# eather0056/Catenary-Model-Estimation-and-MPC-Control-for-ROV-Tethered-Systems

Measured on AMD Instinct MI355X. Metric: MPC rollouts/sec (horizon-steps/sec) at N=20, K=4096; 1/2/4/8 GPU, higher is better.
Workload: dtype f64

## Files before the change

### catenary-model-estimation-and-mpc-control-for-rov-tethered-systems_amd/csrc/rollout_kernels.h

```cpp
#pragma once
#include "device_math.h"

namespace rovmpc {

constexpr int MODEL_BUILTIN = 0;
constexpr int MODEL_INTERP  = 1;
constexpr int MODEL_JIT     = 2;

#ifndef ROVMPC_JIT_FMAP
#define ROVMPC_JIT_FMAP 0
#endif
#ifndef ROVMPC_JIT_N
#define ROVMPC_JIT_N 0
#endif
#ifndef ROVMPC_JIT_CKC
#define ROVMPC_JIT_CKC 0
#endif
#ifndef ROVMPC_JIT_USED
#define ROVMPC_JIT_USED 0xffffffffu
#endif

#ifndef ROVMPC_JIT_NSUB
#define ROVMPC_JIT_NSUB 0
#endif
// ... 61 lines not shown
    int ck_shift;
    unsigned used_planes;
    unsigned magic_3n;
    unsigned long long *granules;
    unsigned epoch;
    int sweeper;
    double *result;
    long long *slots;
    long long k_offset;
    int rank, world;
    unsigned long long *stamps;
    unsigned long long samp_seed, samp_step;
    double samp_mean[3], samp_std[3];
    const double *samp_warm;
    double *samp_best;
    double *samp_blk_u;
    double samp_state[ROVMPC_STATE_LEN];
    T *gtab;
    unsigned long long *gtab_tag;
};


template <typename T>
RV_DEV T interp_eval(const int32_t *__restrict__ code, int n, const T *__restrict__ consts,
                     const T *feat, int fstride, T *stack, int sstride) {
    T top = T(0);
    int sp = 0;
    for (int pc = 0; pc < n; ++pc) {
        int ins = code[pc];
        int op = ins & 0xff, arg = ins >> 8;
        switch (op) {
// ... 27 lines not shown
        case ROVMPC_OP_SAFE_LOG: top = m_log(m_abs(top) + T(1e-5)); break;
        case ROVMPC_OP_SAFE_SQRT: top = m_sqrt(m_abs(top)); break;
        default: top = m_nan<T>(); break;
        }
    }
    return top;
}

constexpr unsigned ERR_WAIT_ROLLED = 1;
constexpr unsigned ERR_CONSUMED    = 2;
constexpr unsigned ERR_SWEEP       = 4;
RV_DEV void raise_error(unsigned *err, unsigned bit) {
    if (err) __hip_atomic_fetch_or(err, bit, __ATOMIC_RELAXED, __HIP_MEMORY_SCOPE_SYSTEM);
}

RV_DEV void st_agent(double *p, double v) { __hip_atomic_store(p, v, __ATOMIC_RELAXED, __HIP_MEMORY_SCOPE_AGENT); }
RV_DEV void st_agent(long long *p, long long v) { __hip_atomic_store(p, v, __ATOMIC_RELAXED, __HIP_MEMORY_SCOPE_AGENT); }
RV_DEV void st_agent(unsigned long long *p, unsigned long long v) { __hip_atomic_store(p, v, __ATOMIC_RELAXED, __HIP_MEMORY_SCOPE_AGENT); }
RV_DEV unsigned long long ld_agent(const unsigned long long *p) { return __hip_atomic_load(p, __ATOMIC_RELAXED, __HIP_MEMORY_SCOPE_AGENT); }
constexpr int GRAN = 4;
RV_DEV void publish_traj_ready(unsigned long long *granules, int nblocks, unsigned epoch) {
    st_agent(granules + 3 * (size_t)nblocks + blockIdx.x, (unsigned long long)epoch << 32);
}
RV_DEV void publish_best(unsigned long long *granules, int nblocks, unsigned epoch, double cost, unsigned lane) {
    const unsigned long long bits = (unsigned long long)__double_as_longlong(cost), tag = (unsigned long long)epoch << 32;
    st_agent(granules + blockIdx.x, tag | (bits >> 32));
    st_agent(granules + nblocks + blockIdx.x, tag | (bits & 0xffffffffULL));
    st_agent(granules + 2 * (size_t)nblocks + blockIdx.x, tag | lane);
}
RV_DEV double ld_agent(const double *p) { return __hip_atomic_load(p, __ATOMIC_RELAXED, __HIP_MEMORY_SCOPE_AGENT); }
RV_DEV float ld_agent(const float *p) { return __hip_atomic_load(p, __ATOMIC_RELAXED, __HIP_MEMORY_SCOPE_AGENT); }
RV_DEV void st_agent(float *p, float v) { __hip_atomic_store(p, v, __ATOMIC_RELAXED, __HIP_MEMORY_SCOPE_AGENT); }
RV_DEV long long ld_agent(const long long *p) { return __hip_atomic_load(p, __ATOMIC_RELAXED, __HIP_MEMORY_SCOPE_AGENT); }

template <typename T, bool LEAN = false, bool SAMPLE = false>
RV_DEV void argmin_epilogue(const RolloutArgs<T> &a, const unsigned long long *granules, const double *blk_traj, const T *U,
                            double *result, double *scratch) {
    const int nblocks = a.nblocks, N = a.N, CK = a.CK, NT = a.NT, rank = a.rank, world = a.world;
    long long *slots = a.slots;
    const unsigned epoch = a.epoch;
    double *sJ = scratch;
    long long *sK = reinterpret_cast<long long *>(scratch + 8);
    const int tid = threadIdx.x, nw = (NT + 63) >> 6;
    double Jd = __builtin_inf();
    long long kk = 0x7fffffffffffffffLL;
    auto take = [&](double oJ, long long ok) {
        const bool better = (oJ < Jd) | ((oJ == Jd) & (ok < kk));
        Jd = better ? oJ : Jd; kk = better ? ok : kk;
    };
    {
        int j = 0;
        const unsigned long long give_up = wall_clock64() + (a.ring ? a.handoff_ticks : 6000000000ULL);
        for (unsigned it = 1;; ++it) {
            bool pending = false;
            for (;;) {
                const int b = tid + j * NT;
                if (b >= nblocks) break;
                const unsigned long long g0 = ld_agent(granules + b), g1 = ld_agent(granules + nblocks + b),
                                         g2 = ld_agent(granules + 2 * (size_t)nblocks + b);
                if ((unsigned)(g0 >> 32) != epoch || (unsigned)(g1 >> 32) != epoch || (unsigned)(g2 >> 32) != epoch) { pending = true; break; }
                const double cost = __longlong_as_double((long long)((g0 << 32) | (g1 & 0xffffffffULL)));
                take(cost, (long long)b * CK + (long long)(g2 & 0xffffffffULL));
                ++j;
            }
            if (!__syncthreads_or(pending)) break;
            if ((it & 1023u) == 0 && __syncthreads_or(wall_clock64() > give_up)) {
                Jd = __builtin_nan(""); kk = 0;
                if (tid == 0) raise_error(a.err, ERR_SWEEP);
                break;
            }
            __builtin_amdgcn_s_sleep(4);
        }
    }
    for (int off = 32; off > 0; off >>= 1) take(__shfl_down(Jd, off, 64), __shfl_down(kk, off, 64));
    if ((tid & 63) == 0) { sJ[tid >> 6] = Jd; sK[tid >> 6] = kk; }
    __syncthreads();
    if (tid == 0) {
        for (int w = 1; w < nw; ++w)
            if (sJ[w] < Jd || (sJ[w] == Jd && sK[w] < kk)) { Jd = sJ[w]; kk = sK[w]; }
        sK[0] = kk;
        sJ[0] = Jd;
    }
    __syncthreads();
    const long long kbest = sK[0];
    const double Jbest = sJ[0];
    const int R = 5 + 2 * (N + 1);
    const double *bt = blk_traj + (size_t)(kbest / CK) * (N + 1) * 2;
    if (Jbest == Jbest) {
        if (tid == 0) {
            const unsigned long long *f = granules + 3 * (size_t)nblocks + (size_t)(kbest / CK);
            const unsigned long long give_up = wall_clock64() + (a.ring ? a.handoff_ticks : 6000000000ULL);
            while ((unsigned)(ld_agent(f) >> 32) != epoch) {
                if (wall_clock64() > give_up) { raise_error(a.err, ERR_SWEEP); break; }
                __builtin_amdgcn_s_sleep(1);
            }
        }
        __syncthreads();
    }
    if (!LEAN && a.ring && a.publish && !slots && tid < 64) {
        if (a.plant_feedback && tid < 4) st_agent(&a.ring[(int)((a.step + 1) & 3) * 4 + tid], ld_agent(&bt[tid < 2 ? 2 + tid : tid - 2]));
        asm volatile("s_waitcnt vmcnt(0)" ::: "memory");
        if (tid == 0) st_agent(a.seq_theta, (unsigned long long)(a.step + 1));
    }
    if (SAMPLE) {
        const double *bu = a.samp_blk_u + (size_t)(kbest / CK) * 3 * N;
        for (int j = tid; j < 3 * N; j += NT) a.samp_best[j] = ld_agent(&bu[j]);
        __syncthreads();
    }
    bool row_free = true;
    if (!LEAN && a.flag_consumed) {
        int *s_ok = reinterpret_cast<int *>(scratch + 15);
        if (tid == 0) {
            const unsigned long long give_up = wall_clock64() + a.handoff_ticks;
            bool ok = true;
            while (ld_agent(a.flag_consumed) < a.consumed_need) {
                if (wall_clock64() > give_up) { ok = false; break; }
                __builtin_amdgcn_s_sleep(8);
            }
            if (!ok) { raise_error(a.err, ERR_CONSUMED); st_agent(a.slot_bad, a.rolled_seq); }
            *s_ok = ok ? 1 : 0;
        }
        __syncthreads();
        row_free = *s_ok != 0;
    }
    for (int i = tid; i < R; i += NT) {
        double v;
        if (i == 0) v = row_free ? Jbest : __builtin_nan("");
        else if (i == 1) v = (double)(kbest + a.k_offset);
        else if (i < 5) v = SAMPLE ? a.samp_best[i - 2] : (double)U[(size_t)kbest * N * 3 + (i - 2)];
        else v = ld_agent(&bt[i - 5]);
        result[i] = v;
        if (!LEAN && a.result_host) a.result_host[i] = v;
        if (!LEAN && slots && row_free) st_agent(&slots[(size_t)rank * R + i], ordered_key(v));
    }
    if (!LEAN && slots && row_free) {
        for (int i = tid; i < world * R; i += NT)
            if (i / R != rank) st_agent(&slots[i], 0x7fffffffffffffffLL);
    }
    if (!LEAN && a.done_flag) {
        asm volatile("s_waitcnt vmcnt(0)" ::: "memory");
        __syncthreads();
        if (tid == 0) {
            __builtin_amdgcn_fence(__ATOMIC_RELEASE, "");
            __hip_atomic_store(a.done_flag, a.done_seq, __ATOMIC_RELEASE, __HIP_MEMORY_SCOPE_SYSTEM);
        }
    }
    if (!LEAN && a.flag_rolled && !(a.inject & 1)) {
        asm volatile("s_waitcnt vmcnt(0)" ::: "memory");
        __syncthreads();
        if (tid == 0) st_agent(a.flag_rolled, a.rolled_seq);
    }
    if (!LEAN && a.plant_next && !(a.ring && slots) && tid < 16) {
        const double *plant_next = a.plant_next;
        double *plant_state = a.plant_state;
        if (!a.plant_feedback) {
            plant_state[tid] = plant_next[tid];
        } else if (tid < 12) {
            plant_state[tid] = plant_next[tid];
        } else if (tid == 12) {
            const double th = a.ring ? ld_agent(&bt[0]) : plant_state[12], ga = a.ring ? ld_agent(&bt[1]) : plant_state[13];
            plant_state[14] = th; plant_state[15] = ga;
            plant_state[12] = ld_agent(&bt[2]); plant_state[13] = ld_agent(&bt[3]);
        }
    }
}


RV_DEV void theta_slot_mark(double *p) { __hip_atomic_store(reinterpret_cast<unsigned long long *>(p), 0x7ff85ea71e5007e7ull, __ATOMIC_RELAXED, __HIP_MEMORY_SCOPE_WORKGROUP); }
RV_DEV void theta_slot_mark(float *p) { __hip_atomic_store(reinterpret_cast<unsigned int *>(p), 0x7fc5ea71u, __ATOMIC_RELAXED, __HIP_MEMORY_SCOPE_WORKGROUP); }
RV_DEV bool theta_slot_marked(double *p) { return __hip_atomic_load(reinterpret_cast<unsigned long long *>(p), __ATOMIC_RELAXED, __HIP_MEMORY_SCOPE_WORKGROUP) == 0x7ff85ea71e5007e7ull; }
RV_DEV bool theta_slot_marked(float *p) { return __hip_atomic_load(reinterpret_cast<unsigned int *>(p), __ATOMIC_RELAXED, __HIP_MEMORY_SCOPE_WORKGROUP) == 0x7fc5ea71u; }

#ifdef ROVMPC_STAMPS
#define RV_STAMP(i) do { if (threadIdx.x == 0 && a.stamps) a.stamps[((size_t)blockIdx.y * gridDim.x + blockIdx.x) * 16 + (i)] = wall_clock64(); } while (0)
#define RV_STAMP_W(i) do { if ((threadIdx.x & 63) == 0 && a.stamps) a.stamps[((size_t)blockIdx.y * gridDim.x + blockIdx.x) * 16 + (i)] = wall_clock64(); } while (0)
#define RV_STAMP_SIMD(i) do { if ((threadIdx.x & 63) == 0 && a.stamps) atomicOr(&a.stamps[((size_t)blockIdx.y * gridDim.x + blockIdx.x) * 16 + (i)], \
    (unsigned long long)(8u | ((__builtin_amdgcn_s_getreg((31 << 11) | 4) >> 4) & 3u)) << (4 * (threadIdx.x >> 6))); } while (0)
#define RV_STAMP_HW(i) do { if (threadIdx.x == 0 && a.stamps) a.stamps[((size_t)blockIdx.y * gridDim.x + blockIdx.x) * 16 + (i)] = \
    (unsigned long long)__builtin_amdgcn_s_getreg((31 << 11) | 4) | ((unsigned long long)__builtin_amdgcn_s_getreg((31 << 11) | 20) << 32); } while (0)
#else
#define RV_STAMP(i) do { } while (0)
#define RV_STAMP_HW(i) do { } while (0)
#define RV_STAMP_SIMD(i) do { } while (0)
#define RV_STAMP_W(i) do { } while (0)
#endif

#define RV_PL(base, p, n, c) (base)[((p) * (N + 1) + (n)) * CK + (c)]
#define RV_PX(s, n, c) RV_PL(sX, xpl(s), n, c)

__host__ __device__ inline int popcount14(unsigned used) {
    int n = 0;
    for (int s = 0; s < NEXO; ++s) n += (used >> s) & 1u;
    return n;
}
__host__ __device__ inline unsigned jit_lds_planes(unsigned used, int vt, int fmap) {
    if (vt != ROVMPC_VT_COMPOSE) return used;
    return fmap == ROVMPC_FEATURES_GEN3 ? 0u : used & ~0x21f8u;
}
__host__ __device__ inline int rollout_nx(int model, int vt, unsigned used = 0xffffffffu) {
    if (model == MODEL_BUILTIN) return vt == ROVMPC_VT_COMPOSE ? 0 : 1;
// ... 1253 lines not shown
            const int n = j >> cks;
            while (__hip_atomic_load(&s_prog[1], __ATOMIC_ACQUIRE, __HIP_MEMORY_SCOPE_WORKGROUP) < n + 1) __builtin_amdgcn_s_sleep(8);
            geometry_b_item(n, j & ckm);
        }
    }
    __syncthreads();

    RV_STAMP(4);
    for (int i = early + tid; i < ((a.debug & 2) ? 0 : N * CK); i += NT) geometry_b_item(i >> cks, i & ckm);
    __syncthreads();

    RV_STAMP(5);
    T *Jb = a.J + (size_t)prob * K;
    T *trajb = a.traj_all ? a.traj_all + (size_t)prob * K * (N + 1) * 2 : nullptr;
    double *blk_trajb = a.blk_traj + (size_t)prob * a.nblocks * (N + 1) * 2;
    unsigned long long *granb = a.granules + (size_t)prob * GRAN * a.nblocks;
    double *resultb = a.result ? a.result + (size_t)prob * (5 + 2 * (N + 1)) : nullptr;
    const bool fast_tail = resultb && !a.traj_all && N + 1 <= 64;
    double &s_best_J = *reinterpret_cast<double *>(reinterpret_cast<char *>(smem) + 16);
    if (tid < 64) {
        const int c = tid;
        double Jd = __builtin_inf();
        long long kk = 0x7fffffffffffffffLL;
        if (c < nvalid) {
            T J = T(0);
            for (int n0 = 0; n0 < N; n0 += 10) {
                T v[10];
#pragma unroll
                for (int e = 0; e < 10; ++e) v[e] = sC[min(n0 + e, N - 1) * CK + c];
#pragma unroll
                for (int e = 0; e < 10; ++e) J = J + (n0 + e < N ? v[e] : T(0));
// ... 5 lines not shown
        auto take = [&](double oJ, long long ok) {
            const bool better = (oJ < Jd) | ((oJ == Jd) & (ok < kk));
            Jd = better ? oJ : Jd; kk = better ? ok : kk;
        };
        if (CK <= 16) {
            take(row_shl<8>(Jd), row_shl<8>(kk));
            take(row_shl<4>(Jd), row_shl<4>(kk));
            take(row_shl<2>(Jd), row_shl<2>(kk));
            take(row_shl<1>(Jd), row_shl<1>(kk));
        } else {
            for (int off = 32; off > 0; off >>= 1) take(__shfl_down(Jd, off, 64), __shfl_down(kk, off, 64));
        }
        if (c == 0) *s_best_c = (int)(kk - k0);
        if (fast_tail) {
            const int cb = __builtin_amdgcn_readfirstlane((int)(kk - k0));
            double *bt = blk_trajb + (size_t)blockIdx.x * (N + 1) * 2;
            if (c <= N) {
                st_agent(&bt[2 * c], (double)RV_PL(sY, 0, c, cb));
                st_agent(&bt[2 * c + 1], (double)RV_PL(sY, 1, c, cb));
            }
            if (SAMPLE) {
                double *bu = a.samp_blk_u + (size_t)blockIdx.x * 3 * N;
                for (int j = c; j < 3 * N; j += 64) st_agent(&bu[j], (double)sU[cb * US + j]);
            }
            if (c == 0) publish_best(granb, a.nblocks, a.epoch, Jd, (unsigned)cb);
            asm volatile("s_waitcnt vmcnt(0)" ::: "memory");
            if (c == 0) publish_traj_ready(granb, a.nblocks, a.epoch);
        } else if (c == 0) {
            s_best_J = Jd;
        }
    }
    RV_STAMP(14);
    __syncthreads();
    RV_STAMP(15);
    if (!fast_tail) {
        const int cb = *s_best_c;
        double *bt = blk_trajb + (size_t)blockIdx.x * (N + 1) * 2;
        for (int i = tid; i < (N + 1); i += NT) {
            st_agent(&bt[2 * i], (double)RV_PL(sY, 0, i, cb));
            st_agent(&bt[2 * i + 1], (double)RV_PL(sY, 1, i, cb));
        }
        if (SAMPLE) {
            double *bu = a.samp_blk_u + (size_t)blockIdx.x * 3 * N;
            for (int j = tid; j < 3 * N; j += NT) st_agent(&bu[j], (double)sU[cb * US + j]);
        }
        if (trajb) {
            for (int i = tid; i < nvalid * (N + 1); i += NT) {
                const int c = i / (N + 1), n = i % (N + 1);
                T *dst = trajb + ((size_t)(k0 + c) * (N + 1) + n) * 2;
                dst[0] = RV_PL(sY, 0, n, c); dst[1] = RV_PL(sY, 1, n, c);
            }
        }
    }
    RV_STAMP(6);
    if (!resultb) return;
    if (!fast_tail) {

    asm volatile("s_waitcnt vmcnt(0)" ::: "memory");
    __syncthreads();
    if (tid == 0) { publish_best(granb, a.nblocks, a.epoch, s_best_J, (unsigned)*s_best_c); publish_traj_ready(granb, a.nblocks, a.epoch); }
    }
    RV_STAMP(7);
    if ((int)blockIdx.x != a.sweeper) return;
    if (HANDOFF) {
        argmin_epilogue<T>(a, granb, blk_trajb, Ub, resultb, reinterpret_cast<double *>(smem + 4));
    } else if (LEAN) {
        argmin_epilogue<T, true>(a, granb, blk_trajb, Ub, resultb, reinterpret_cast<double *>(smem + 4));
    } else if (SAMPLE) {
        argmin_epilogue<T, false, true>(a, granb, blk_trajb, Ub, resultb, reinterpret_cast<double *>(smem + 4));
    } else {
#if defined(__HIP_DEVICE_COMPILE__)
        const RolloutArgs<T> *ap = (const RolloutArgs<T> *)__builtin_amdgcn_kernarg_segment_ptr();
        asm volatile("" : "+s"(ap));
#else
        const RolloutArgs<T> *ap = &a;
#endif
        argmin_epilogue<T>(*ap, granb, blk_trajb, Ub, resultb, reinterpret_cast<double *>(smem + 4));
    }
}

template <typename T, int MODEL, int VT>
__global__ void __launch_bounds__(512)
rollout_kernel(const RolloutArgs<T> a) {
    rollout_body<T, MODEL, VT>(a);
}

template <typename T, int MODEL, int VT>
__global__ void __launch_bounds__(512)
rollout_kernel_long(const RolloutArgs<T> a) {
    rollout_body<T, MODEL, VT, false, false, false, true>(a);
}

// ... 60 lines not shown
struct HandoffArgs {
    long long T;
    const double *exo;
    unsigned long long *seq_theta;
    unsigned long long *seq_gamma;
    double *ring;
    unsigned long long *granules2;
    double *blk_traj2;
    long long step;
};

template <typename T, int MODEL, int VT, int CKC = 0, int NC = 0>
RV_DEV void closed_loop_step_body(const RolloutArgs<T> &a0, const HandoffArgs &p) {
    const long long g = p.step;
    RolloutArgs<T> a = a0;
    a.granules = p.granules2 + (size_t)(g & 1) * GRAN * a0.nblocks;
    a.blk_traj = p.blk_traj2 + (size_t)(g & 1) * a0.nblocks * (a0.N + 1) * 2;
    a.exo_cur = p.exo + (size_t)g * ROVMPC_STATE_LEN;
    a.ring = p.ring; a.seq_theta = p.seq_theta; a.seq_gamma = p.seq_gamma;
    a.step = g;
    a.from_ring = a0.plant_feedback && g > 0;
    a.wait_theta = a.from_ring;
    a.publish = g + 1 < p.T;
    a.plant_next = g + 1 < p.T ? p.exo + (size_t)(g + 1) * ROVMPC_STATE_LEN : nullptr;
    a.plant_state = const_cast<double *>(a0.state);
    rollout_body<T, MODEL, VT, true, false, false, false, CKC, NC>(a);
}

template <typename T, int MODEL, int VT>
__global__ void __launch_bounds__(512)
closed_loop_step_kernel(const RolloutArgs<T> a, const HandoffArgs p) {
// ... 91 lines not shown
```

### catenary-model-estimation-and-mpc-control-for-rov-tethered-systems_amd/csrc/rovmpc.hip

```cpp
#include <hip/hip_runtime.h>
#include <math.h>
#include <stdio.h>
#include <stdlib.h>
#include <string.h>
#include <string>
#include <vector>

#include <hip/hiprtc.h>
#include <rccl/rccl.h>
#include <dlfcn.h>
#include <chrono>
#include <condition_variable>
#include <deque>
#include <map>
#include <mutex>
#include <thread>

#include "util_kernels.h"
#include "cem_kernels.h"
#include "embedded_sources.inc"

using namespace rovmpc;

static thread_local std::string g_create_error;
// ... 71 lines not shown
    unsigned *epoch_ctr = nullptr;
    unsigned long long *d_stamps = nullptr;
    void *d_gtab = nullptr;
    const unsigned long long *arg_flag_consumed = nullptr;
    unsigned long long *arg_flag_rolled = nullptr;
    unsigned long long arg_consumed_need = 0, arg_rolled_seq = 0;
    unsigned long long *arg_slot_bad = nullptr;
    int arg_inject = 0;
    unsigned *h_err = nullptr, *d_err = nullptr;
    double handoff_timeout_ms = 10000.0;
    int inject_skip_rolled = 0, inject_skip_consumed = 0;
    void *d_Us[2] = {nullptr, nullptr};
    Mailbox samp_box;
    unsigned long long samp_steps = 0;
    double *d_best = nullptr;
    double *d_blk_u = nullptr;
    unsigned long long last_seed = 0, last_step = 0; double last_mean[3] = {}, last_std[3] = {}; int last_warm = 0; bool last_fused = false;
    double *arg_result_host = nullptr; unsigned long long *arg_done_flag = nullptr; unsigned long long arg_done_seq = 0;
    void *arg_J = nullptr;
    PlanCtl mppi{"MPPI", "mppi", "MPPI step"}, cem{"CEM", "cem", "CEM step"};
    PlanBatch mppi_b{"MPPI", "mppi"}, cem_b{"CEM", "cem"};
    int batch_cap = 0, last_batch = 1;
    void *d_Jb = nullptr; double *d_blk_trajb = nullptr; unsigned long long *d_granulesb = nullptr;
    const double *plant_next = nullptr;
    double *plant_state = nullptr;
    int plant_feedback = 0;
    double *h_result = nullptr;
    ncclComm_t comm = nullptr;
    int comm_rank = 0, comm_world = 0, comm_flip = 0;
    static constexpr int NSLOT = 4;
    static constexpr int NCOMM_MAX = 3;
// ... 314 lines not shown
    CR(hipStreamCreateWithFlags(&h->stream, hipStreamNonBlocking));
    h->pipe_streams[1] = process_pipe_stream(cfg->device);
    const size_t R = 5 + 2 * (size_t)(cfg->N + 1);
    CR(hipMalloc(&h->d_U, (size_t)cfg->K * cfg->N * 3 * h->esz));
    CR(hipMalloc(&h->d_J, (size_t)cfg->K * h->esz));
    CR(hipMalloc((void **)&h->d_state, ROVMPC_STATE_LEN * sizeof(double)));
    CR(hipMalloc((void **)&h->d_blk_traj, (size_t)max_blocks * (cfg->N + 1) * 2 * sizeof(double)));
    CR(hipMalloc((void **)&h->d_result, R * sizeof(double)));
    CR(hipHostMalloc((void **)&h->h_result, R * sizeof(double), hipHostMallocDefault));
    CR(hipMalloc((void **)&h->d_code_th, ROVMPC_MAX_CODE * sizeof(int32_t)));
    CR(hipMalloc((void **)&h->d_code_ga, ROVMPC_MAX_CODE * sizeof(int32_t)));
    CR(hipMalloc(&h->d_consts, ROVMPC_MAX_CODE * 8));
    CR(hipMalloc((void **)&h->d_consts64, ROVMPC_MAX_CODE * 8));
    CR(hipMalloc(&h->d_Rtab, (size_t)cfg->N * 9 * h->esz));
    CR(hipMalloc(&h->d_k, sizeof(RolloutConsts<double>)));
    CR(hipMalloc((void **)&h->d_granules, (size_t)GRAN * max_blocks * sizeof(unsigned long long)));
    CR(hipMemset(h->d_granules, 0, (size_t)GRAN * max_blocks * sizeof(unsigned long long)));
    h->epoch_ctr = new unsigned(0);
    CR(hipMalloc(&h->d_gtab, (size_t)8 * (cfg->N + 1) * 8 + 64));
    CR(hipMemset(h->d_gtab, 0, (size_t)8 * (cfg->N + 1) * 8 + 64));
    CR(hipHostMalloc((void **)&h->h_err, 64, hipHostMallocMapped));
    *h->h_err = 0;
    CR(hipHostGetDevicePointer((void **)&h->d_err, h->h_err, 0));
#ifdef ROVMPC_STAMPS
    CR(hipMalloc((void **)&h->d_stamps, (size_t)max_blocks * 16 * sizeof(unsigned long long)));
    CR(hipMemset(h->d_stamps, 0, (size_t)max_blocks * 16 * sizeof(unsigned long long)));
#endif
#undef CR
    *out = h;
    return ROVMPC_OK;
}

extern "C" int rovmpc_comm_destroy(rovmpc_handle *h);

extern "C" void rovmpc_destroy(rovmpc_handle *h) {
    if (!h) return;
    (void)rovmpc_comm_destroy(h);
    (void)hipSetDevice(h->cfg.device);
    if (h->stream) (void)hipStreamSynchronize(h->stream);
    for (auto &e : h->ev) (void)hipEventDestroy(e);
    void *ptrs[] = {h->d_U, h->d_J, h->d_traj_all, h->d_state, h->d_blk_traj,
// ... 519 lines not shown
    if (time_it) { HIPCHK(h, hipEventRecord(h->ev[h->ev_used + 1], s)); h->ev_used += 2; }
    return ROVMPC_OK;
}

extern "C" int rovmpc_step_device(rovmpc_handle *h, const double *d_state, const void *d_U, double *d_result, void *stream) {
    if (!h) return ROVMPC_ERR_INVALID;
    if (!d_state || !d_U || !d_result) FAIL(h, ROVMPC_ERR_INVALID, "rovmpc_step_device: null pointer");
    return enqueue_step(h, d_state, d_U, nullptr, d_result, 0, nullptr, 0, 1, (hipStream_t)stream);
}

static int ensure_batch(rovmpc_handle *h, int B) {
    if (B <= h->batch_cap) return ROVMPC_OK;
    HIPCHK(h, hipSetDevice(h->cfg.device));
    const rovmpc_config &c = h->cfg;
    const size_t max_blocks = c.candidates_per_block > 0 ? (size_t)((c.K + c.candidates_per_block - 1) / c.candidates_per_block) : (size_t)c.K;
    const size_t gran_bytes = (size_t)B * GRAN * max_blocks * sizeof(unsigned long long);
    void *fresh[3] = {nullptr, nullptr, nullptr};
    hipError_t e = hipMalloc(&fresh[0], (size_t)B * c.K * h->esz);
    if (e == hipSuccess) e = hipMalloc(&fresh[1], (size_t)B * max_blocks * (c.N + 1) * 2 * sizeof(double));
    if (e == hipSuccess) e = hipMalloc(&fresh[2], gran_bytes);
    if (e == hipSuccess) e = hipMemset(fresh[2], 0, gran_bytes);
    if (e == hipSuccess) e = hipDeviceSynchronize();
    if (e != hipSuccess) {
        for (void *p : fresh) if (p) (void)hipFree(p);
        (void)hipGetLastError();
        FAIL(h, ROVMPC_ERR_HIP, "batched workspace for %d problems: %s", B, hipGetErrorString(e));
    }
    void *old[] = {h->d_Jb, h->d_blk_trajb, h->d_granulesb};
    for (void *p : old) if (p) (void)hipFree(p);
    h->d_Jb = fresh[0]; h->d_blk_trajb = (double *)fresh[1]; h->d_granulesb = (unsigned long long *)fresh[2];
    h->batch_cap = B;
// ... 118 lines not shown
    int rc = check_ready(h);
    if (rc) return rc;
    HIPCHK(h, hipSetDevice(h->cfg.device));
    if ((rc = ensure_sampler(h))) return rc;
    const int cur = (int)(h->samp_steps & 1);
    const int warm = warm_start && h->samp_steps > 0;
    const bool fused = h->model_kind == MODEL_BUILTIN && (h->samp_steps == 0 || h->last_fused) && !h->timing;
    const bool prev_fused = h->samp_steps > 0 && h->last_fused;
    h->last_seed = seed; h->last_step = step; h->last_warm = warm; h->last_fused = fused;
    for (int i = 0; i < 3; ++i) { h->last_mean[i] = mean3[i]; h->last_std[i] = std3[i]; }
    unsigned long long seq = h->samp_steps + 1;
    if (fused) {
        if (!h->d_best) {
            const size_t max_blocks = h->cfg.candidates_per_block > 0 ? (size_t)((h->cfg.K + h->cfg.candidates_per_block - 1) / h->cfg.candidates_per_block) : (size_t)h->cfg.K;
            HIPCHK(h, hipMalloc((void **)&h->d_best, (size_t)2 * h->cfg.N * 3 * sizeof(double)));
            HIPCHK(h, hipMalloc((void **)&h->d_blk_u, max_blocks * (size_t)h->cfg.N * 3 * sizeof(double)));
        }
        rc = h->cfg.dtype == ROVMPC_F64 ? fused_sampled_step_t<double>(h, state, seed, step, mean3, std3, warm, seq)
                                        : fused_sampled_step_t<float>(h, state, seed, step, mean3, std3, warm, seq);
        ++h->samp_steps;
        if (rc) return rc;
    } else {
    const double *warm_seq = (warm && prev_fused) ? h->d_best + (size_t)(cur ^ 1) * h->cfg.N * 3 : nullptr;
    if ((rc = launch_sampler(h, state, seed, step, mean3, std3, warm, h->d_Us[cur], h->d_Us[cur ^ 1], h->stream, warm_seq))) return rc;
    seq = ++h->samp_steps;
    h->arg_result_host = h->samp_box.d_out; h->arg_done_flag = h->samp_box.d_done; h->arg_done_seq = seq;
    rc = enqueue_step(h, h->d_state, h->d_Us[cur], nullptr, h->d_result, 0, nullptr, 0, 1, h->stream);
    h->arg_result_host = nullptr; h->arg_done_flag = nullptr;
    if (rc) return rc;
    }
    if ((rc = mailbox_wait(h, h->samp_box, seq, "step"))) return rc;
// ... 991 lines not shown
    if (n == 0) return ROVMPC_OK;
    HIPCHK(h, hipSetDevice(h->cfg.device));
    DevBuf dR, dv, dout;
    UPLOAD(h, dR, R, (size_t)n * 9 * sizeof(double));
    UPLOAD(h, dv, v, (size_t)n * 3 * sizeof(double));
    HIPCHK(h, dout.alloc((size_t)n * 3 * sizeof(double)));
    hipLaunchKernelGGL(velocity_transform_kernel, dim3(grid_for(n, 256)), dim3(256), 0, h->stream, dR.as<double>(), dv.as<double>(),
                       (long long)n, dout.as<double>());
    HIPCHK(h, hipGetLastError());
    HIPCHK(h, hipMemcpyAsync(out, dout.p, (size_t)n * 3 * sizeof(double), hipMemcpyDeviceToHost, h->stream));
    HIPCHK(h, hipStreamSynchronize(h->stream));
    return ROVMPC_OK;
}

#ifdef ROVMPC_STAMPS
extern "C" int rovmpc_diag_read_stamps(rovmpc_handle *h, unsigned long long *out, int32_t *nblocks) {
    if (!h || !out) return ROVMPC_ERR_INVALID;
    HIPCHK(h, hipSetDevice(h->cfg.device));
    HIPCHK(h, hipDeviceSynchronize());
    HIPCHK(h, hipMemcpy(out, h->d_stamps, (size_t)h->nblocks * 16 * sizeof(unsigned long long), hipMemcpyDeviceToHost));
    HIPCHK(h, hipMemset(h->d_stamps, 0, (size_t)h->nblocks * 16 * sizeof(unsigned long long)));
    if (nblocks) *nblocks = h->nblocks;
    return ROVMPC_OK;
}
#endif

extern "C" int rovmpc_extract_features(rovmpc_handle *h, const double *P0, const double *P1, const double *V1, const double *time,
                                       const double *theta, const double *gamma, int64_t T, int32_t with_prev, double *out) {
    if (!h) return ROVMPC_ERR_INVALID;
    if (T < 2 || !P0 || !P1 || !V1 || !time || !theta || !gamma || !out)
        FAIL(h, ROVMPC_ERR_INVALID, "rovmpc_extract_features: bad argument (np.gradient needs at least 2 rows)");
    HIPCHK(h, hipSetDevice(h->cfg.device));
    const int F = with_prev ? 18 : 16;
    DevBuf d0, d1, dv, dt, dth, dga, dout;
    UPLOAD(h, d0, P0, (size_t)T * 3 * sizeof(double));
    UPLOAD(h, d1, P1, (size_t)T * 3 * sizeof(double));
// ... 498 lines not shown
        for (int d = c; d < rovmpc_handle::NCOMM_MAX; ++d)
            if (h->comm_streams[d] == st) h->comm_streams[d] = nullptr;
        (void)hipStreamDestroy(st);
    }
    h->comm_placed = false;
    h->comm_aborted = false;
    return take_device_errors(h);
}


static int closed_loop_workspace(rovmpc_handle *h, HandoffArgs &p, hipStream_t s) {
    const rovmpc_config &c = h->cfg;
    const size_t max_blocks = c.candidates_per_block > 0 ? (size_t)((c.K + c.candidates_per_block - 1) / c.candidates_per_block) : (size_t)c.K;
    if (!h->d_step_seq) {
        HIPCHK(h, hipMalloc((void **)&h->d_step_seq, 256));
        HIPCHK(h, hipMalloc((void **)&h->d_cl_granules, 2 * GRAN * max_blocks * sizeof(unsigned long long)));
        HIPCHK(h, hipMemset(h->d_cl_granules, 0, 2 * GRAN * max_blocks * sizeof(unsigned long long)));
        HIPCHK(h, hipMalloc((void **)&h->d_cl_blk_traj, 2 * max_blocks * (size_t)(c.N + 1) * 2 * sizeof(double)));
    }
    HIPCHK(h, hipMemsetAsync(h->d_step_seq, 0, 128, s));
    HIPCHK(h, hipMemsetAsync(h->d_step_seq + 16, 0xff, 128, s));
    p.seq_theta = h->d_step_seq; p.seq_gamma = h->d_step_seq + 8;
    p.ring = reinterpret_cast<double *>(h->d_step_seq + 16);
    p.granules2 = h->d_cl_granules; p.blk_traj2 = h->d_cl_blk_traj;
    return ROVMPC_OK;
}

template <typename T, int VT>
static hipError_t launch_step(const rovmpc_handle *h, const RolloutArgs<T> &a, const HandoffArgs &p, hipStream_t s, bool probe, int *capacity) {
    const size_t lds = rollout_lds_elems<T>(a.N, a.CK, MODEL_BUILTIN, VT) * sizeof(T);
    auto kern = (a.CK == 16 && a.ck_shift == 4) ? closed_loop_step_kernel16<T, MODEL_BUILTIN, VT> : closed_loop_step_kernel<T, MODEL_BUILTIN, VT>;
    if constexpr (sizeof(T) == 8) { if (a.CK == 16 && a.ck_shift == 4 && a.N == 20 && !getenv("ROVMPC_NO_LITERAL_N")) kern = closed_loop_step_kernel16_n20<T, MODEL_BUILTIN, VT>; }
// ... 263 lines not shown
```

Baseline: 5.387 billion.

## Tag per-block winner trajectory with epoch and use single-wave argmin sweep

Each block now publishes its best trajectory and sampled controls as epoch-tagged 32-bit halves, so the sweeper can read the winner's data directly without waiting on a separate traj-ready flag and its vmcnt drain. For grids of 256 blocks or fewer, the argmin sweep runs in a single wave with unrolled granule loads, ballot-based polling and DPP row shifts, which removes block-wide syncs. In the lean path the other waves exit early. The costs are a larger granule buffer, doubled store traffic for tagged values, and per-element polling when the winner is read.

```diff
diff --git a/catenary-model-estimation-and-mpc-control-for-rov-tethered-systems_amd/csrc/rollout_kernels.h b/catenary-model-estimation-and-mpc-control-for-rov-tethered-systems_amd/csrc/rollout_kernels.h
--- a/catenary-model-estimation-and-mpc-control-for-rov-tethered-systems_amd/csrc/rollout_kernels.h
+++ b/catenary-model-estimation-and-mpc-control-for-rov-tethered-systems_amd/csrc/rollout_kernels.h
@@ -99,7 +99,7 @@
     double samp_mean[3], samp_std[3];
     const double *samp_warm;
     double *samp_best;
-    double *samp_blk_u;
+    unsigned long long *samp_blk_u;
     double samp_state[ROVMPC_STATE_LEN];
     T *gtab;
     unsigned long long *gtab_tag;
@@ -157,11 +157,30 @@
     if (err) __hip_atomic_fetch_or(err, bit, __ATOMIC_RELAXED, __HIP_MEMORY_SCOPE_SYSTEM);
 }
 
+#ifdef ROVMPC_STAMPS
+#define RV_NSTAMP 24
+#define RV_STAMP(i) do { if (threadIdx.x == 0 && a.stamps) a.stamps[((size_t)blockIdx.y * gridDim.x + blockIdx.x) * RV_NSTAMP + (i)] = wall_clock64(); } while (0)
+#define RV_STAMP_W(i) do { if ((threadIdx.x & 63) == 0 && a.stamps) a.stamps[((size_t)blockIdx.y * gridDim.x + blockIdx.x) * RV_NSTAMP + (i)] = wall_clock64(); } while (0)
+#define RV_STAMP_SIMD(i) do { if ((threadIdx.x & 63) == 0 && a.stamps) atomicOr(&a.stamps[((size_t)blockIdx.y * gridDim.x + blockIdx.x) * RV_NSTAMP + (i)], \
+    (unsigned long long)(8u | ((__builtin_amdgcn_s_getreg((31 << 11) | 4) >> 4) & 3u)) << (4 * (threadIdx.x >> 6))); } while (0)
+#define RV_STAMP_HW(i) do { if (threadIdx.x == 0 && a.stamps) a.stamps[((size_t)blockIdx.y * gridDim.x + blockIdx.x) * RV_NSTAMP + (i)] = \
+    (unsigned long long)__builtin_amdgcn_s_getreg((31 << 11) | 4) | ((unsigned long long)__builtin_amdgcn_s_getreg((31 << 11) | 20) << 32); } while (0)
+#define RV_STAMP_T(i, t) do { if (threadIdx.x == (t) && a.stamps) { asm volatile("s_waitcnt vmcnt(0)" ::: "memory"); \
+    a.stamps[((size_t)blockIdx.y * gridDim.x + blockIdx.x) * RV_NSTAMP + (i)] = wall_clock64(); } } while (0)
+#else
+#define RV_STAMP(i) do { } while (0)
+#define RV_STAMP_T(i, t) do { } while (0)
+#define RV_STAMP_HW(i) do { } while (0)
+#define RV_STAMP_SIMD(i) do { } while (0)
+#define RV_STAMP_W(i) do { } while (0)
+#endif
+
 RV_DEV void st_agent(double *p, double v) { __hip_atomic_store(p, v, __ATOMIC_RELAXED, __HIP_MEMORY_SCOPE_AGENT); }
 RV_DEV void st_agent(long long *p, long long v) { __hip_atomic_store(p, v, __ATOMIC_RELAXED, __HIP_MEMORY_SCOPE_AGENT); }
 RV_DEV void st_agent(unsigned long long *p, unsigned long long v) { __hip_atomic_store(p, v, __ATOMIC_RELAXED, __HIP_MEMORY_SCOPE_AGENT); }
 RV_DEV unsigned long long ld_agent(const unsigned long long *p) { return __hip_atomic_load(p, __ATOMIC_RELAXED, __HIP_MEMORY_SCOPE_AGENT); }
 constexpr int GRAN = 4;
+__host__ __device__ inline size_t gran_stride(int nblocks, int N) { return (size_t)nblocks * (size_t)(GRAN + 4 * (N + 1)); }
 RV_DEV void publish_traj_ready(unsigned long long *granules, int nblocks, unsigned epoch) {
     st_agent(granules + 3 * (size_t)nblocks + blockIdx.x, (unsigned long long)epoch << 32);
 }
@@ -172,13 +191,33 @@
     st_agent(granules + 2 * (size_t)nblocks + blockIdx.x, tag | lane);
 }
 RV_DEV double ld_agent(const double *p) { return __hip_atomic_load(p, __ATOMIC_RELAXED, __HIP_MEMORY_SCOPE_AGENT); }
+RV_DEV void st_tagged(unsigned long long *g, unsigned epoch, double v) {
+    const unsigned long long bits = (unsigned long long)__double_as_longlong(v), tag = (unsigned long long)epoch << 32;
+    st_agent(g, tag | (bits >> 32));
+    st_agent(g + 1, tag | (bits & 0xffffffffULL));
+}
+RV_DEV double ld_tagged(const unsigned long long *g, unsigned epoch, bool wait, unsigned long long ticks, unsigned *err) {
+    unsigned long long g0 = ld_agent(g), g1 = ld_agent(g + 1);
+    if ((unsigned)(g0 >> 32) != epoch || (unsigned)(g1 >> 32) != epoch) {
+        const unsigned long long give_up = wall_clock64() + ticks;
+        for (;;) {
+            if (!wait) return __builtin_nan("");
+            if ((unsigned)(g0 >> 32) != epoch) g0 = ld_agent(g);
+            if ((unsigned)(g1 >> 32) != epoch) g1 = ld_agent(g + 1);
+            if ((unsigned)(g0 >> 32) == epoch && (unsigned)(g1 >> 32) == epoch) break;
+            if (wall_clock64() > give_up) { raise_error(err, ERR_SWEEP); return __builtin_nan(""); }
+            __builtin_amdgcn_s_sleep(1);
+        }
+    }
+    return __longlong_as_double((long long)((g0 << 32) | (g1 & 0xffffffffULL)));
+}
 RV_DEV float ld_agent(const float *p) { return __hip_atomic_load(p, __ATOMIC_RELAXED, __HIP_MEMORY_SCOPE_AGENT); }
 RV_DEV void st_agent(float *p, float v) { __hip_atomic_store(p, v, __ATOMIC_RELAXED, __HIP_MEMORY_SCOPE_AGENT); }
 RV_DEV long long ld_agent(const long long *p) { return __hip_atomic_load(p, __ATOMIC_RELAXED, __HIP_MEMORY_SCOPE_AGENT); }
 
 template <typename T, bool LEAN = false, bool SAMPLE = false>
-RV_DEV void argmin_epilogue(const RolloutArgs<T> &a, const unsigned long long *granules, const double *blk_traj, const T *U,
-                            double *result, double *scratch) {
+RV_DEV void argmin_epilogue(const RolloutArgs<T> &a, const unsigned long long *granules, const double *blk_traj, const bool tagged,
+                            const T *U, double *result, double *scratch) {
     const int nblocks = a.nblocks, N = a.N, CK = a.CK, NT = a.NT, rank = a.rank, world = a.world;
     long long *slots = a.slots;
     const unsigned epoch = a.epoch;
@@ -191,45 +230,108 @@
         const bool better = (oJ < Jd) | ((oJ == Jd) & (ok < kk));
         Jd = better ? oJ : Jd; kk = better ? ok : kk;
     };
-    {
-        int j = 0;
-        const unsigned long long give_up = wall_clock64() + (a.ring ? a.handoff_ticks : 6000000000ULL);
-        for (unsigned it = 1;; ++it) {
-            bool pending = false;
-            for (;;) {
-                const int b = tid + j * NT;
-                if (b >= nblocks) break;
-                const unsigned long long g0 = ld_agent(granules + b), g1 = ld_agent(granules + nblocks + b),
-                                         g2 = ld_agent(granules + 2 * (size_t)nblocks + b);
-                if ((unsigned)(g0 >> 32) != epoch || (unsigned)(g1 >> 32) != epoch || (unsigned)(g2 >> 32) != epoch) { pending = true; break; }
-                const double cost = __longlong_as_double((long long)((g0 << 32) | (g1 & 0xffffffffULL)));
-                take(cost, (long long)b * CK + (long long)(g2 & 0xffffffffULL));
-                ++j;
-            }
-            if (!__syncthreads_or(pending)) break;
-            if ((it & 1023u) == 0 && __syncthreads_or(wall_clock64() > give_up)) {
-                Jd = __builtin_nan(""); kk = 0;
-                if (tid == 0) raise_error(a.err, ERR_SWEEP);
-                break;
-            }
-            __builtin_amdgcn_s_sleep(4);
-        }
-    }
-    for (int off = 32; off > 0; off >>= 1) take(__shfl_down(Jd, off, 64), __shfl_down(kk, off, 64));
-    if ((tid & 63) == 0) { sJ[tid >> 6] = Jd; sK[tid >> 6] = kk; }
-    __syncthreads();
-    if (tid == 0) {
-        for (int w = 1; w < nw; ++w)
-            if (sJ[w] < Jd || (sJ[w] == Jd && sK[w] < kk)) { Jd = sJ[w]; kk = sK[w]; }
-        sK[0] = kk;
-        sJ[0] = Jd;
-    }
-    __syncthreads();
-    const long long kbest = sK[0];
-    const double Jbest = sJ[0];
+    const bool small = nblocks <= 256;
+    const bool solo = LEAN && small && tagged;
+    if (small) {
+        if (solo && tid >= 64) return;
+        if (tid < 64) {
+            const unsigned long long give_up = wall_clock64() + (a.ring ? a.handoff_ticks : 6000000000ULL);
+            bool gave_up = false;
+            for (unsigned it = 1;; ++it) {
+                unsigned long long g0[4], g1[4], g2[4];
+#pragma unroll
+                for (int q = 0; q < 4; ++q) {
+                    const int b = min(tid + 64 * q, nblocks - 1);
+                    g0[q] = ld_agent(granules + b); g1[q] = ld_agent(granules + nblocks + b); g2[q] = ld_agent(granules + 2 * (size_t)nblocks + b);
+                }
+                Jd = __builtin_inf(); kk = 0x7fffffffffffffffLL;
+                bool pending = false;
+#pragma unroll
+                for (int q = 0; q < 4; ++q) {
+                    const int b = tid + 64 * q;
+                    const bool ok = (unsigned)(g0[q] >> 32) == epoch && (unsigned)(g1[q] >> 32) == epoch && (unsigned)(g2[q] >> 32) == epoch;
+                    pending |= (b < nblocks) & !ok;
+                    const double cost = __longlong_as_double((long long)((g0[q] << 32) | (g1[q] & 0xffffffffULL)));
+                    const bool use = (b < nblocks) & ok;
+                    take(use ? cost : __builtin_inf(), use ? (long long)b * CK + (long long)(g2[q] & 0xffffffffULL) : 0x7fffffffffffffffLL);
+                }
+                if (__builtin_amdgcn_ballot_w64(pending) == 0) break;
+                if ((it & 1023u) == 0 && __builtin_amdgcn_ballot_w64(wall_clock64() > give_up) != 0) {
+                    gave_up = true;
+                    if (tid == 0) raise_error(a.err, ERR_SWEEP);
+                    break;
+                }
+                __builtin_amdgcn_s_sleep(2);
+            }
+            RV_STAMP(16);
+            take(__shfl_down(Jd, 32, 64), __shfl_down(kk, 32, 64));
+            take(__shfl_down(Jd, 16, 64), __shfl_down(kk, 16, 64));
+            take(row_shl<8>(Jd), row_shl<8>(kk));
+            take(row_shl<4>(Jd), row_shl<4>(kk));
+            take(row_shl<2>(Jd), row_shl<2>(kk));
+            take(row_shl<1>(Jd), row_shl<1>(kk));
+            if (gave_up) { Jd = __builtin_nan(""); kk = 0; }
+            if (solo) {
+                const unsigned long long jb = (unsigned long long)__double_as_longlong(Jd), kb = (unsigned long long)kk;
+                const unsigned jl = __builtin_amdgcn_readfirstlane((int)(unsigned)jb), jh = __builtin_amdgcn_readfirstlane((int)(unsigned)(jb >> 32));
+                const unsigned kl = __builtin_amdgcn_readfirstlane((int)(unsigned)kb), kh = __builtin_amdgcn_readfirstlane((int)(unsigned)(kb >> 32));
+                Jd = __longlong_as_double((long long)(((unsigned long long)jh << 32) | jl));
+                kk = (long long)(((unsigned long long)kh << 32) | kl);
+            } else if (tid == 0) {
+                sJ[0] = Jd; sK[0] = kk;
+            }
+        }
+        if (!solo) {
+            __syncthreads();
+            Jd = sJ[0]; kk = sK[0];
+        }
+    } else {
+        {
+            int j = 0;
+            const unsigned long long give_up = wall_clock64() + (a.ring ? a.handoff_ticks : 6000000000ULL);
+            for (unsigned it = 1;; ++it) {
+                bool pending = false;
+                for (;;) {
+                    const int b = tid + j * NT;
+                    if (b >= nblocks) break;
+                    const unsigned long long g0 = ld_agent(granules + b), g1 = ld_agent(granules + nblocks + b),
+                                             g2 = ld_agent(granules + 2 * (size_t)nblocks + b);
+                    if ((unsigned)(g0 >> 32) != epoch || (unsigned)(g1 >> 32) != epoch || (unsigned)(g2 >> 32) != epoch) { pending = true; break; }
+                    const double cost = __longlong_as_double((long long)((g0 << 32) | (g1 & 0xffffffffULL)));
+                    take(cost, (long long)b * CK + (long long)(g2 & 0xffffffffULL));
+                    ++j;
+                }
+                if (!__syncthreads_or(pending)) break;
+                if ((it & 1023u) == 0 && __syncthreads_or(wall_clock64() > give_up)) {
+                    Jd = __builtin_nan(""); kk = 0;
+                    if (tid == 0) raise_error(a.err, ERR_SWEEP);
+                    break;
+                }
+                __builtin_amdgcn_s_sleep(4);
+            }
+        }
+        RV_STAMP(16);
+        take(__shfl_down(Jd, 32, 64), __shfl_down(kk, 32, 64));
+        take(__shfl_down(Jd, 16, 64), __shfl_down(kk, 16, 64));
+        take(row_shl<8>(Jd), row_shl<8>(kk));
+        take(row_shl<4>(Jd), row_shl<4>(kk));
+        take(row_shl<2>(Jd), row_shl<2>(kk));
+        take(row_shl<1>(Jd), row_shl<1>(kk));
+        if ((tid & 63) == 0) { sJ[tid >> 6] = Jd; sK[tid >> 6] = kk; }
+        __syncthreads();
+        Jd = sJ[0]; kk = sK[0];
+        for (int w = 1; w < nw; ++w) take(sJ[w], sK[w]);
+    }
+    const long long kbest = kk;
+    const double Jbest = Jd;
+    RV_STAMP(17);
     const int R = 5 + 2 * (N + 1);
     const double *bt = blk_traj + (size_t)(kbest / CK) * (N + 1) * 2;
-    if (Jbest == Jbest) {
+    const unsigned long long *tg = granules + (size_t)GRAN * nblocks + (size_t)(kbest / CK) * 4 * (N + 1);
+    const bool have = Jbest == Jbest;
+    const unsigned long long tail_ticks = a.ring ? a.handoff_ticks : 6000000000ULL;
+    auto winner = [&](int i) -> double { return tagged ? ld_tagged(tg + 2 * i, epoch, have, tail_ticks, a.err) : ld_agent(&bt[i]); };
+    if (!tagged && have) {
         if (tid == 0) {
             const unsigned long long *f = granules + 3 * (size_t)nblocks + (size_t)(kbest / CK);
             const unsigned long long give_up = wall_clock64() + (a.ring ? a.handoff_ticks : 6000000000ULL);
@@ -239,20 +341,23 @@
             }
         }
         __syncthreads();
+        RV_STAMP(20);
     }
     if (!LEAN && a.ring && a.publish && !slots && tid < 64) {
-        if (a.plant_feedback && tid < 4) st_agent(&a.ring[(int)((a.step + 1) & 3) * 4 + tid], ld_agent(&bt[tid < 2 ? 2 + tid : tid - 2]));
+        if (a.plant_feedback && tid < 4) st_agent(&a.ring[(int)((a.step + 1) & 3) * 4 + tid], winner(tid < 2 ? 2 + tid : tid - 2));
         asm volatile("s_waitcnt vmcnt(0)" ::: "memory");
         if (tid == 0) st_agent(a.seq_theta, (unsigned long long)(a.step + 1));
     }
     if (SAMPLE) {
-        const double *bu = a.samp_blk_u + (size_t)(kbest / CK) * 3 * N;
-        for (int j = tid; j < 3 * N; j += NT) a.samp_best[j] = ld_agent(&bu[j]);
+        const unsigned long long *bug = a.samp_blk_u + (size_t)(kbest / CK) * 6 * N;
+        const double *bu = reinterpret_cast<const double *>(a.samp_blk_u + (size_t)nblocks * 6 * N) + (size_t)(kbest / CK) * 3 * N;
+        for (int j = tid; j < 3 * N; j += NT) a.samp_best[j] = tagged ? ld_tagged(bug + 2 * j, epoch, have, tail_ticks, a.err) : ld_agent(&bu[j]);
         __syncthreads();
     }
     bool row_free = true;
     if (!LEAN && a.flag_consumed) {
         int *s_ok = reinterpret_cast<int *>(scratch + 15);
+        __syncthreads();
         if (tid == 0) {
             const unsigned long long give_up = wall_clock64() + a.handoff_ticks;
             bool ok = true;
@@ -266,16 +371,18 @@
         __syncthreads();
         row_free = *s_ok != 0;
     }
-    for (int i = tid; i < R; i += NT) {
+    for (int i = tid; i < R; i += (solo ? 64 : NT)) {
         double v;
         if (i == 0) v = row_free ? Jbest : __builtin_nan("");
         else if (i == 1) v = (double)(kbest + a.k_offset);
         else if (i < 5) v = SAMPLE ? a.samp_best[i - 2] : (double)U[(size_t)kbest * N * 3 + (i - 2)];
-        else v = ld_agent(&bt[i - 5]);
+        else v = winner(i - 5);
+        RV_STAMP_T(18, 5);
         result[i] = v;
         if (!LEAN && a.result_host) a.result_host[i] = v;
         if (!LEAN && slots && row_free) st_agent(&slots[(size_t)rank * R + i], ordered_key(v));
     }
+    RV_STAMP_T(19, 5);
     if (!LEAN && slots && row_free) {
         for (int i = tid; i < world * R; i += NT)
             if (i / R != rank) st_agent(&slots[i], 0x7fffffffffffffffLL);
@@ -301,9 +408,9 @@
         } else if (tid < 12) {
             plant_state[tid] = plant_next[tid];
         } else if (tid == 12) {
-            const double th = a.ring ? ld_agent(&bt[0]) : plant_state[12], ga = a.ring ? ld_agent(&bt[1]) : plant_state[13];
+            const double th = a.ring ? winner(0) : plant_state[12], ga = a.ring ? winner(1) : plant_state[13];
             plant_state[14] = th; plant_state[15] = ga;
-            plant_state[12] = ld_agent(&bt[2]); plant_state[13] = ld_agent(&bt[3]);
+            plant_state[12] = winner(2); plant_state[13] = winner(3);
         }
     }
 }
@@ -313,20 +420,6 @@
 RV_DEV void theta_slot_mark(float *p) { __hip_atomic_store(reinterpret_cast<unsigned int *>(p), 0x7fc5ea71u, __ATOMIC_RELAXED, __HIP_MEMORY_SCOPE_WORKGROUP); }
 RV_DEV bool theta_slot_marked(double *p) { return __hip_atomic_load(reinterpret_cast<unsigned long long *>(p), __ATOMIC_RELAXED, __HIP_MEMORY_SCOPE_WORKGROUP) == 0x7ff85ea71e5007e7ull; }
 RV_DEV bool theta_slot_marked(float *p) { return __hip_atomic_load(reinterpret_cast<unsigned int *>(p), __ATOMIC_RELAXED, __HIP_MEMORY_SCOPE_WORKGROUP) == 0x7fc5ea71u; }
-
-#ifdef ROVMPC_STAMPS
-#define RV_STAMP(i) do { if (threadIdx.x == 0 && a.stamps) a.stamps[((size_t)blockIdx.y * gridDim.x + blockIdx.x) * 16 + (i)] = wall_clock64(); } while (0)
-#define RV_STAMP_W(i) do { if ((threadIdx.x & 63) == 0 && a.stamps) a.stamps[((size_t)blockIdx.y * gridDim.x + blockIdx.x) * 16 + (i)] = wall_clock64(); } while (0)
-#define RV_STAMP_SIMD(i) do { if ((threadIdx.x & 63) == 0 && a.stamps) atomicOr(&a.stamps[((size_t)blockIdx.y * gridDim.x + blockIdx.x) * 16 + (i)], \
-    (unsigned long long)(8u | ((__builtin_amdgcn_s_getreg((31 << 11) | 4) >> 4) & 3u)) << (4 * (threadIdx.x >> 6))); } while (0)
-#define RV_STAMP_HW(i) do { if (threadIdx.x == 0 && a.stamps) a.stamps[((size_t)blockIdx.y * gridDim.x + blockIdx.x) * 16 + (i)] = \
-    (unsigned long long)__builtin_amdgcn_s_getreg((31 << 11) | 4) | ((unsigned long long)__builtin_amdgcn_s_getreg((31 << 11) | 20) << 32); } while (0)
-#else
-#define RV_STAMP(i) do { } while (0)
-#define RV_STAMP_HW(i) do { } while (0)
-#define RV_STAMP_SIMD(i) do { } while (0)
-#define RV_STAMP_W(i) do { } while (0)
-#endif
 
 #define RV_PL(base, p, n, c) (base)[((p) * (N + 1) + (n)) * CK + (c)]
 #define RV_PX(s, n, c) RV_PL(sX, xpl(s), n, c)
@@ -1610,7 +1703,7 @@
     T *Jb = a.J + (size_t)prob * K;
     T *trajb = a.traj_all ? a.traj_all + (size_t)prob * K * (N + 1) * 2 : nullptr;
     double *blk_trajb = a.blk_traj + (size_t)prob * a.nblocks * (N + 1) * 2;
-    unsigned long long *granb = a.granules + (size_t)prob * GRAN * a.nblocks;
+    unsigned long long *granb = a.granules + (size_t)prob * gran_stride(a.nblocks, N);
     double *resultb = a.result ? a.result + (size_t)prob * (5 + 2 * (N + 1)) : nullptr;
     const bool fast_tail = resultb && !a.traj_all && N + 1 <= 64;
     double &s_best_J = *reinterpret_cast<double *>(reinterpret_cast<char *>(smem) + 16);
@@ -1646,18 +1739,16 @@
         if (c == 0) *s_best_c = (int)(kk - k0);
         if (fast_tail) {
             const int cb = __builtin_amdgcn_readfirstlane((int)(kk - k0));
-            double *bt = blk_trajb + (size_t)blockIdx.x * (N + 1) * 2;
+            if (c == 0) publish_best(granb, a.nblocks, a.epoch, Jd, (unsigned)cb);
+            unsigned long long *tg = granb + (size_t)GRAN * a.nblocks + (size_t)blockIdx.x * 4 * (N + 1);
             if (c <= N) {
-                st_agent(&bt[2 * c], (double)RV_PL(sY, 0, c, cb));
-                st_agent(&bt[2 * c + 1], (double)RV_PL(sY, 1, c, cb));
+                st_tagged(tg + 4 * c, a.epoch, (double)RV_PL(sY, 0, c, cb));
+                st_tagged(tg + 4 * c + 2, a.epoch, (double)RV_PL(sY, 1, c, cb));
             }
             if (SAMPLE) {
-                double *bu = a.samp_blk_u + (size_t)blockIdx.x * 3 * N;
-                for (int j = c; j < 3 * N; j += 64) st_agent(&bu[j], (double)sU[cb * US + j]);
-            }
-            if (c == 0) publish_best(granb, a.nblocks, a.epoch, Jd, (unsigned)cb);
-            asm volatile("s_waitcnt vmcnt(0)" ::: "memory");
-            if (c == 0) publish_traj_ready(granb, a.nblocks, a.epoch);
+                unsigned long long *bu = a.samp_blk_u + (size_t)blockIdx.x * 6 * N;
+                for (int j = c; j < 3 * N; j += 64) st_tagged(bu + 2 * j, a.epoch, (double)sU[cb * US + j]);
+            }
         } else if (c == 0) {
             s_best_J = Jd;
         }
@@ -1673,7 +1764,7 @@
             st_agent(&bt[2 * i + 1], (double)RV_PL(sY, 1, i, cb));
         }
         if (SAMPLE) {
-            double *bu = a.samp_blk_u + (size_t)blockIdx.x * 3 * N;
+            double *bu = reinterpret_cast<double *>(a.samp_blk_u + (size_t)a.nblocks * 6 * N) + (size_t)blockIdx.x * 3 * N;
             for (int j = tid; j < 3 * N; j += NT) st_agent(&bu[j], (double)sU[cb * US + j]);
         }
         if (trajb) {
@@ -1695,11 +1786,11 @@
     RV_STAMP(7);
     if ((int)blockIdx.x != a.sweeper) return;
     if (HANDOFF) {
-        argmin_epilogue<T>(a, granb, blk_trajb, Ub, resultb, reinterpret_cast<double *>(smem + 4));
+        argmin_epilogue<T>(a, granb, blk_trajb, fast_tail, Ub, resultb, reinterpret_cast<double *>(smem + 4));
     } else if (LEAN) {
-        argmin_epilogue<T, true>(a, granb, blk_trajb, Ub, resultb, reinterpret_cast<double *>(smem + 4));
+        argmin_epilogue<T, true>(a, granb, blk_trajb, fast_tail, Ub, resultb, reinterpret_cast<double *>(smem + 4));
     } else if (SAMPLE) {
-        argmin_epilogue<T, false, true>(a, granb, blk_trajb, Ub, resultb, reinterpret_cast<double *>(smem + 4));
+        argmin_epilogue<T, false, true>(a, granb, blk_trajb, fast_tail, Ub, resultb, reinterpret_cast<double *>(smem + 4));
     } else {
 #if defined(__HIP_DEVICE_COMPILE__)
         const RolloutArgs<T> *ap = (const RolloutArgs<T> *)__builtin_amdgcn_kernarg_segment_ptr();
@@ -1707,7 +1798,7 @@
 #else
         const RolloutArgs<T> *ap = &a;
 #endif
-        argmin_epilogue<T>(*ap, granb, blk_trajb, Ub, resultb, reinterpret_cast<double *>(smem + 4));
+        argmin_epilogue<T>(*ap, granb, blk_trajb, fast_tail, Ub, resultb, reinterpret_cast<double *>(smem + 4));
     }
 }
 
@@ -1798,7 +1889,7 @@
 RV_DEV void closed_loop_step_body(const RolloutArgs<T> &a0, const HandoffArgs &p) {
     const long long g = p.step;
     RolloutArgs<T> a = a0;
-    a.granules = p.granules2 + (size_t)(g & 1) * GRAN * a0.nblocks;
+    a.granules = p.granules2 + (size_t)(g & 1) * gran_stride(a0.nblocks, a0.N);
     a.blk_traj = p.blk_traj2 + (size_t)(g & 1) * a0.nblocks * (a0.N + 1) * 2;
     a.exo_cur = p.exo + (size_t)g * ROVMPC_STATE_LEN;
     a.ring = p.ring; a.seq_theta = p.seq_theta; a.seq_gamma = p.seq_gamma;
diff --git a/catenary-model-estimation-and-mpc-control-for-rov-tethered-systems_amd/csrc/rovmpc.hip b/catenary-model-estimation-and-mpc-control-for-rov-tethered-systems_amd/csrc/rovmpc.hip
--- a/catenary-model-estimation-and-mpc-control-for-rov-tethered-systems_amd/csrc/rovmpc.hip
+++ b/catenary-model-estimation-and-mpc-control-for-rov-tethered-systems_amd/csrc/rovmpc.hip
@@ -109,7 +109,7 @@
     Mailbox samp_box;
     unsigned long long samp_steps = 0;
     double *d_best = nullptr;
-    double *d_blk_u = nullptr;
+    unsigned long long *d_blk_u = nullptr;
     unsigned long long last_seed = 0, last_step = 0; double last_mean[3] = {}, last_std[3] = {}; int last_warm = 0; bool last_fused = false;
     double *arg_result_host = nullptr; unsigned long long *arg_done_flag = nullptr; unsigned long long arg_done_seq = 0;
     void *arg_J = nullptr;
@@ -454,8 +454,8 @@
     CR(hipMalloc((void **)&h->d_consts64, ROVMPC_MAX_CODE * 8));
     CR(hipMalloc(&h->d_Rtab, (size_t)cfg->N * 9 * h->esz));
     CR(hipMalloc(&h->d_k, sizeof(RolloutConsts<double>)));
-    CR(hipMalloc((void **)&h->d_granules, (size_t)GRAN * max_blocks * sizeof(unsigned long long)));
-    CR(hipMemset(h->d_granules, 0, (size_t)GRAN * max_blocks * sizeof(unsigned long long)));
+    CR(hipMalloc((void **)&h->d_granules, gran_stride((int)max_blocks, cfg->N) * sizeof(unsigned long long)));
+    CR(hipMemset(h->d_granules, 0, gran_stride((int)max_blocks, cfg->N) * sizeof(unsigned long long)));
     h->epoch_ctr = new unsigned(0);
     CR(hipMalloc(&h->d_gtab, (size_t)8 * (cfg->N + 1) * 8 + 64));
     CR(hipMemset(h->d_gtab, 0, (size_t)8 * (cfg->N + 1) * 8 + 64));
@@ -463,8 +463,8 @@
     *h->h_err = 0;
     CR(hipHostGetDevicePointer((void **)&h->d_err, h->h_err, 0));
 #ifdef ROVMPC_STAMPS
-    CR(hipMalloc((void **)&h->d_stamps, (size_t)max_blocks * 16 * sizeof(unsigned long long)));
-    CR(hipMemset(h->d_stamps, 0, (size_t)max_blocks * 16 * sizeof(unsigned long long)));
+    CR(hipMalloc((void **)&h->d_stamps, (size_t)max_blocks * RV_NSTAMP * sizeof(unsigned long long)));
+    CR(hipMemset(h->d_stamps, 0, (size_t)max_blocks * RV_NSTAMP * sizeof(unsigned long long)));
 #endif
 #undef CR
     *out = h;
@@ -1014,7 +1014,7 @@
     HIPCHK(h, hipSetDevice(h->cfg.device));
     const rovmpc_config &c = h->cfg;
     const size_t max_blocks = c.candidates_per_block > 0 ? (size_t)((c.K + c.candidates_per_block - 1) / c.candidates_per_block) : (size_t)c.K;
-    const size_t gran_bytes = (size_t)B * GRAN * max_blocks * sizeof(unsigned long long);
+    const size_t gran_bytes = (size_t)B * gran_stride((int)max_blocks, c.N) * sizeof(unsigned long long);
     void *fresh[3] = {nullptr, nullptr, nullptr};
     hipError_t e = hipMalloc(&fresh[0], (size_t)B * c.K * h->esz);
     if (e == hipSuccess) e = hipMalloc(&fresh[1], (size_t)B * max_blocks * (c.N + 1) * 2 * sizeof(double));
@@ -1163,7 +1163,8 @@
         if (!h->d_best) {
             const size_t max_blocks = h->cfg.candidates_per_block > 0 ? (size_t)((h->cfg.K + h->cfg.candidates_per_block - 1) / h->cfg.candidates_per_block) : (size_t)h->cfg.K;
             HIPCHK(h, hipMalloc((void **)&h->d_best, (size_t)2 * h->cfg.N * 3 * sizeof(double)));
-            HIPCHK(h, hipMalloc((void **)&h->d_blk_u, max_blocks * (size_t)h->cfg.N * 3 * sizeof(double)));
+            HIPCHK(h, hipMalloc((void **)&h->d_blk_u, max_blocks * (size_t)h->cfg.N * 9 * sizeof(unsigned long long)));
+            HIPCHK(h, hipMemset(h->d_blk_u, 0, max_blocks * (size_t)h->cfg.N * 9 * sizeof(unsigned long long)));
         }
         rc = h->cfg.dtype == ROVMPC_F64 ? fused_sampled_step_t<double>(h, state, seed, step, mean3, std3, warm, seq)
                                         : fused_sampled_step_t<float>(h, state, seed, step, mean3, std3, warm, seq);
@@ -2185,12 +2186,13 @@
 }
 
 #ifdef ROVMPC_STAMPS
+extern "C" int32_t rovmpc_diag_stamp_slots(void) { return RV_NSTAMP; }
 extern "C" int rovmpc_diag_read_stamps(rovmpc_handle *h, unsigned long long *out, int32_t *nblocks) {
     if (!h || !out) return ROVMPC_ERR_INVALID;
     HIPCHK(h, hipSetDevice(h->cfg.device));
     HIPCHK(h, hipDeviceSynchronize());
-    HIPCHK(h, hipMemcpy(out, h->d_stamps, (size_t)h->nblocks * 16 * sizeof(unsigned long long), hipMemcpyDeviceToHost));
-    HIPCHK(h, hipMemset(h->d_stamps, 0, (size_t)h->nblocks * 16 * sizeof(unsigned long long)));
+    HIPCHK(h, hipMemcpy(out, h->d_stamps, (size_t)h->nblocks * RV_NSTAMP * sizeof(unsigned long long), hipMemcpyDeviceToHost));
+    HIPCHK(h, hipMemset(h->d_stamps, 0, (size_t)h->nblocks * RV_NSTAMP * sizeof(unsigned long long)));
     if (nblocks) *nblocks = h->nblocks;
     return ROVMPC_OK;
 }
@@ -2719,8 +2721,8 @@
     const size_t max_blocks = c.candidates_per_block > 0 ? (size_t)((c.K + c.candidates_per_block - 1) / c.candidates_per_block) : (size_t)c.K;
     if (!h->d_step_seq) {
         HIPCHK(h, hipMalloc((void **)&h->d_step_seq, 256));
-        HIPCHK(h, hipMalloc((void **)&h->d_cl_granules, 2 * GRAN * max_blocks * sizeof(unsigned long long)));
-        HIPCHK(h, hipMemset(h->d_cl_granules, 0, 2 * GRAN * max_blocks * sizeof(unsigned long long)));
+        HIPCHK(h, hipMalloc((void **)&h->d_cl_granules, 2 * gran_stride((int)max_blocks, c.N) * sizeof(unsigned long long)));
+        HIPCHK(h, hipMemset(h->d_cl_granules, 0, 2 * gran_stride((int)max_blocks, c.N) * sizeof(unsigned long long)));
         HIPCHK(h, hipMalloc((void **)&h->d_cl_blk_traj, 2 * max_blocks * (size_t)(c.N + 1) * 2 * sizeof(double)));
     }
     HIPCHK(h, hipMemsetAsync(h->d_step_seq, 0, 128, s));
```

Measured after the change: 5.920 billion, median of 6. 9.9% higher.
